# madronalabs/madronalib

Measured on AMD Instinct MI355X. Metric: voice-samples/sec (SawGen->SVF chain), higher is better.
Workload: dtype f32

## Files before the change

include/mlgpu.h:

```cpp
#ifndef MLGPU_H
#define MLGPU_H

#ifndef __HIPCC_RTC__
#include <stddef.h>
#endif
#include <stdint.h>

#ifdef __cplusplus
extern "C" {
#endif

#define MLGPU_FLOATS_PER_DSPVECTOR 64
#define MLGPU_ABI_VERSION 2


typedef enum mlgpu_status
{
  MLGPU_OK = 0,
  MLGPU_ERR_INVALID = 1,
  MLGPU_ERR_NO_DEVICE = 2,
  MLGPU_ERR_HIP = 3,
  MLGPU_ERR_OOM = 4,
  MLGPU_ERR_UNSUPPORTED = 5,
  MLGPU_ERR_RANGE = 6,
// ... 270 lines not shown
  const char* name;
  int node_type;
  int kind;
  int n_inputs;
  int n_required_inputs;
  int n_params;
  const char* output_name;
} mlgpu_registry_entry;
int mlgpu_registry_count(void);
int mlgpu_registry_get(int index, mlgpu_registry_entry* out);
int mlgpu_registry_lookup(const char* name, mlgpu_registry_entry* out);
int mlgpu_registry_input_name(const char* name, int index, char* buf, size_t buf_len);
int mlgpu_registry_param_name(const char* name, int index, char* buf, size_t buf_len);
int mlgpu_registry_param_index(const char* name, const char* param);
int mlgpu_graph_add_named(mlgpu_graph* g, const char* proc_name, const char* node_name, const char* const* input_node_names, int n_inputs);
int mlgpu_graph_set_named_coeff(mlgpu_graph* g, const char* node_name, const char* coeff_name, const float* h_per_voice, float uniform);
int mlgpu_graph_set_param_by_name(mlgpu_graph* g, const char* param_name, const float* h_per_voice, float uniform);

int mlgpu_graph_add_output(mlgpu_graph* g, int node);
int mlgpu_graph_node(mlgpu_graph* g, const char* name);
int mlgpu_graph_set_node_name(mlgpu_graph* g, int node, const char* name);
int mlgpu_graph_node_kind(mlgpu_graph* g, int node);
int mlgpu_graph_node_use_count(mlgpu_graph* g, int node);
int mlgpu_graph_num_nodes(mlgpu_graph* g);
int mlgpu_graph_set_voices_per_lane(mlgpu_graph* g, int n);
size_t mlgpu_graph_device_bytes(mlgpu_graph* g);
int mlgpu_graph_set_autotune(mlgpu_graph* g, int on);
int mlgpu_graph_tuning(mlgpu_graph* g, int* voices_per_lane, int* quads_per_trip);
int mlgpu_graph_workgroups_per_cu(mlgpu_graph* g);
int mlgpu_graph_compile(mlgpu_graph* g);
int mlgpu_graph_compile_async(mlgpu_graph* g);
int mlgpu_graph_compile_poll(mlgpu_graph* g);
const char* mlgpu_graph_source(mlgpu_graph* g);
int mlgpu_graph_emit(mlgpu_graph* g, const void** code, size_t* code_size);
const char* mlgpu_graph_last_error(mlgpu_graph* g);
int mlgpu_graph_clear(mlgpu_graph* g);
int mlgpu_graph_clear_proc(mlgpu_graph* g, int proc_node);
int mlgpu_graph_set_state_uniform(mlgpu_graph* g, int proc_node, int state_idx, uint32_t value);
int mlgpu_graph_set_param(mlgpu_graph* g, int param_node, const float* h_per_voice);
int mlgpu_graph_set_param_uniform(mlgpu_graph* g, int param_node, float value);
int mlgpu_graph_num_coeffs(mlgpu_graph* g, int proc_node);
int mlgpu_graph_num_state(mlgpu_graph* g, int proc_node);
int mlgpu_graph_set_coeff(mlgpu_graph* g, int proc_node, int coeff_idx, const float* h_per_voice);
int mlgpu_graph_set_coeff_uniform(mlgpu_graph* g, int proc_node, int coeff_idx, float value);
int mlgpu_graph_get_state(mlgpu_graph* g, int proc_node, int state_idx, uint32_t* h_per_voice);
int mlgpu_graph_set_state(mlgpu_graph* g, int proc_node, int state_idx, const uint32_t* h_per_voice);
int mlgpu_graph_process(mlgpu_graph* g, size_t n_vectors, const float* const* d_inputs, int in_layout,
                        float* const* d_outputs, int out_layout);
int mlgpu_graph_set_input_layout(mlgpu_graph* g, int input_index, int layout);
int mlgpu_graph_process_ctl(mlgpu_graph* g, size_t n_vectors, const float* const* d_inputs, int in_layout,
                            const float* const* d_controls, float* const* d_outputs, int out_layout);

int mlgpu_engine_set_jit(mlgpu_engine* e, int enabled);
int mlgpu_jit_selftest(char* log, size_t log_len);
int mlgpu_jit_stats(uint64_t* compiles, uint64_t* disk_hits, uint64_t* memory_hits, double* compile_seconds, double* disk_load_seconds);
int mlgpu_jit_cache_export(void* buffer, size_t capacity, size_t* needed);
int mlgpu_jit_cache_import(const void* buffer, size_t size, size_t* kernels);
int mlgpu_jit_cache_clear_memory(void);
int mlgpu_jit_compiler_available(void);

typedef enum mlgpu_event_type
{
  MLGPU_EVENT_NULL = 0,
  MLGPU_EVENT_NOTE_ON = 1,
  MLGPU_EVENT_NOTE_RETRIG = 2,
  MLGPU_EVENT_NOTE_SUSTAIN = 3,
// ... 157 lines not shown
```

madronalib_amd/__init__.py:

```python
import ctypes
import weakref

import numpy as np

from . import _lib
from .constants import FLOATS_PER_DSPVECTOR, Layout, Op, Proc, Region, Route, RowOp, RowsRule, Status, Vop

__all__ = ["Engine", "Bank", "Graph", "DSPBuffer", "ProcessBuffer", "Resampler", "Events", "Event", "EventType", "jit_selftest", "DeviceBuffer", "MlgpuError", "Layout", "Op", "Proc", "RowOp", "Status", "Vop", "Route", "RowsRule", "Allpass1", "FractionalDelay", "LinearGlide", "SampleAccurateLinearGlide",
           "Lopass", "Hipass", "Bandpass", "LoShelf", "HiShelf", "Bell", "OnePole", "DCBlocker", "ADSR",
           "dBToGain", "device_count", "FLOATS_PER_DSPVECTOR"]


BUSY = 7


def behaviour_revision():
    return _lib.load().mlgpu_behaviour_revision()


class MlgpuError(RuntimeError):
    def __init__(self, status, detail=""):
        L = _lib.load()
        self.status = status
        super().__init__(f"mlgpu status {status} ({L.mlgpu_status_string(status).decode()}) {detail}")
# ... 1022 lines not shown
    def add_output(self, node):
        self.outputs.append(node)
        self.engine._check(self.L.mlgpu_graph_add_output(self.h, self._id(node)))

    def set_output_group_sum(self, output_index, group):
        self._check(self.L.mlgpu_graph_set_output_group_sum(self.h, int(output_index), int(group)))

    def set_output_mixdown(self, output_index, on=True):
        self._check(self.L.mlgpu_graph_set_output_mixdown(self.h, int(output_index), 2 if on == "shard" else (1 if on else 0)))

    def reserve_mixdown(self, max_vectors):
        self._check(self.L.mlgpu_graph_reserve_mixdown(self.h, int(max_vectors)))

    def set_input_group(self, input_index, group):
        self._check(self.L.mlgpu_graph_set_input_group(self.h, int(input_index), int(group)))

    def compile(self):
        self.engine._check(self.L.mlgpu_graph_compile(self.h))

    def compile_async(self):
        self.engine._check(self.L.mlgpu_graph_compile_async(self.h))

    def compile_poll(self):
        st = self.L.mlgpu_graph_compile_poll(self.h)
        if st == BUSY:
            return False
        self.engine._check(st)
        return True

    @property
    def source(self):
        return self.L.mlgpu_graph_source(self.h).decode()

    def clear(self):
        self.engine._check(self.L.mlgpu_graph_clear(self.h))

    def set_param(self, node, value):
        if np.isscalar(value):
            self.engine._check(self.L.mlgpu_graph_set_param_uniform(self.h, self._id(node), float(value)))
        else:
            v = np.ascontiguousarray(value, np.float32)
            assert v.shape == (self.V,)
            self.engine._check(self.L.mlgpu_graph_set_param(self.h, self._id(node), _np_ptr(v)))

    def set_coeff(self, node, idx, value):
        if np.isscalar(value):
            self.engine._check(self.L.mlgpu_graph_set_coeff_uniform(self.h, self._id(node), idx, float(value)))
        else:
            v = np.ascontiguousarray(value, np.float32)
            assert v.shape == (self.V,)
            self.engine._check(self.L.mlgpu_graph_set_coeff(self.h, self._id(node), idx, _np_ptr(v)))

    def set_coeffs(self, node, coeffs):
        for i, c in enumerate(coeffs):
            self.set_coeff(node, i, c if np.ndim(c) else float(c))

    def num_state(self, node):
        return self.L.mlgpu_graph_num_state(self.h, self._id(node))

    def get_state(self, node, idx):
        out = np.empty(self.V, np.uint32)
        self.engine._check(self.L.mlgpu_graph_get_state(self.h, self._id(node), idx, _np_ptr(out)))
        return out

    def set_state(self, node, idx, value):
        v = np.ascontiguousarray(np.broadcast_to(np.asarray(value, np.uint32), (self.V,)))
# ... 145 lines not shown
```

madronalib_amd/_lib.py:

```python
import ctypes
import os
import subprocess
import threading

HERE = os.path.dirname(os.path.abspath(__file__))
CSRC = os.path.join(HERE, "csrc")
LIB_PATH = os.path.join(CSRC, "libmlgpu.so")
HEADER = os.path.join(os.path.dirname(HERE), "include", "mlgpu.h")

def _sources():
    names = {"Makefile", "embed.py"}
    try:
        text = open(os.path.join(CSRC, "Makefile")).read().replace("\\\n", " ")
        vars_ = {}
        for line in text.splitlines():
            if "=" in line and not line.startswith("\t") and not line.lstrip().startswith("#"):
                k, _, v = line.partition("=")
                vars_[k.strip().rstrip("?:+").strip()] = v.strip()
        for key in ("SRCS", "DEVHDRS", "HDRS"):
            for tok in vars_.get(key, "").split():
                if tok.startswith("$("):
                    continue
                names.add(tok)
    except OSError:
# ... 146 lines not shown
    sig("mlgpu_graph_add_const", i, [vp, f])
    sig("mlgpu_graph_set_live_constants", i, [vp, i])
    sig("mlgpu_graph_set_const", i, [vp, i, f])
    sig("mlgpu_graph_update_constants_from", i, [vp, vp])
    sig("mlgpu_graph_add_const_vector", i, [vp, ctypes.POINTER(ctypes.c_float), ctypes.c_char_p])
    sig("mlgpu_graph_add_control", i, [vp, c.c_char_p])
    sig("mlgpu_graph_add_feedback", i, [vp, c.c_char_p])
    sig("mlgpu_graph_set_feedback", i, [vp, i, i])
    sig("mlgpu_graph_set_max_delay", i, [vp, i, f])
    sig("mlgpu_allpass1_make_coeffs", f, [f])
    sig("mlgpu_fractional_delay_make_state", None, [f, fp])
    sig("mlgpu_graph_add_vop", i, [vp, i, ip, i, c.c_char_p])
    sig("mlgpu_graph_process_ctl", i, [vp, sz, pp, i, pp, pp, i])
    sig("mlgpu_graph_last_error", c.c_char_p, [vp])
    sig("mlgpu_graph_set_output_group_sum", i, [vp, i, i])
    sig("mlgpu_graph_set_output_mixdown", i, [vp, i, i])
    sig("mlgpu_graph_reserve_mixdown", i, [vp, sz])
    sig("mlgpu_graph_set_input_group", i, [vp, i, i])
    sig("mlgpu_graph_add_event_row", i, [vp, i, c.c_char_p])
    sig("mlgpu_graph_bind_events", i, [vp, vp])
    sig("mlgpu_graph_process_events", i, [vp, sz, i, pp, i, pp, pp, i])
    sig("mlgpu_linear_glide_make_coeffs", None, [f, fp])
    sig("mlgpu_sample_accurate_linear_glide_make_coeffs", None, [f, fp])
    sig("mlgpu_graph_add_proc", i, [vp, i, ip, i, c.c_char_p])
    sig("mlgpu_graph_add_op", i, [vp, i, ip, i, c.c_char_p])
    sig("mlgpu_graph_add_output", i, [vp, i])
    sig("mlgpu_graph_node", i, [vp, c.c_char_p])
    sig("mlgpu_graph_num_nodes", i, [vp])
    sig("mlgpu_graph_compile", i, [vp])
    sig("mlgpu_graph_compile_async", i, [vp])
    sig("mlgpu_graph_compile_poll", i, [vp])
    sig("mlgpu_behaviour_revision", i, [])
    sig("mlgpu_graph_source", c.c_char_p, [vp])
    sig("mlgpu_graph_node_use_count", i, [vp, i])
    sig("mlgpu_graph_emit", i, [vp, c.POINTER(vp), c.POINTER(c.c_size_t)])
    sig("mlgpu_graph_begin_region", i, [vp, i, c.POINTER(i), i, c.POINTER(i)])
    sig("mlgpu_graph_end_region", i, [vp, i, c.c_char_p])
    sig("mlgpu_graph_clear", i, [vp])
    sig("mlgpu_graph_clear_proc", i, [vp, i])
    sig("mlgpu_graph_set_input_layout", i, [vp, i, i])
    sig("mlgpu_graph_set_voices_per_lane", i, [vp, i])
    sig("mlgpu_graph_set_delay_layout", i, [vp, i])
    sig("mlgpu_graph_delay_layout", i, [vp])
    sig("mlgpu_graph_device_bytes", sz, [vp])
    sig("mlgpu_graph_set_autotune", i, [vp, i])
    sig("mlgpu_graph_tuning", i, [vp, c.POINTER(i), c.POINTER(i)])
    sig("mlgpu_graph_workgroups_per_cu", i, [vp])
    sig("mlgpu_mixdown_reserve", i, [vp, sz, sz])
    sig("mlgpu_mixdown_shard_level", i, [sz])
    sig("mlgpu_mixdown_shard_rows", sz, [sz])
    sig("mlgpu_mixdown_shard", i, [vp, vp, i, sz, sz, vp, vp])
    sig("mlgpu_bank_process_mixdown_shard", i, [vp, sz, vp, i, vp, vp])
    sig("mlgpu_mixdown_finish", i, [fp, sz, sz, i, fp, fp])
    sig("mlgpu_mixdown", i, [vp, vp, i, sz, sz, vp, vp])
    sig("mlgpu_mixdown_groups", i, [vp, vp, i, sz, sz, sz, vp, i])
    sig("mlgpu_events_create", i, [vp, sz, i, pp])
    sig("mlgpu_events_destroy", i, [vp])
    sig("mlgpu_events_clear", i, [vp])
    sig("mlgpu_events_set_sample_rate", i, [vp, c.c_double])
    sig("mlgpu_events_set_protocol", i, [vp, i])
    sig("mlgpu_events_set_unison", i, [vp, i])
    sig("mlgpu_events_set_mod_cc", i, [vp, i])
    sig("mlgpu_events_set_pitch_bend_semitones", i, [vp, f])
    sig("mlgpu_events_set_mpe_pitch_bend_semitones", i, [vp, f])
    sig("mlgpu_events_set_pitch_glide_seconds", i, [vp, f])
    sig("mlgpu_events_set_drift_amount", i, [vp, f])
# ... 80 lines not shown
```

madronalib_amd/csrc/graph.hip:

```cpp
#include <math.h>
#include <stdio.h>
#include <stdlib.h>
#include <string.h>

#include <algorithm>
#include <atomic>
#include <thread>
#include <mutex>
#include <new>
#include <set>

#include "graph_codegen.hpp"
#include "mlgpu_internal.hpp"

using namespace mlgraph;

struct mlgpu_graph;
static std::mutex g_boundMutex;
static std::set<mlgpu_graph*> g_boundGraphs;

namespace
{
int opArity(int op) { return op >= 64 ? 3 : (op >= 32 ? 2 : 1); }
bool opKnown(int op)
// ... 771 lines not shown
    {
      err = allocate(g->d_consts, (size_t)(g->desc.nConsts + 1));
      for (const Node& n : g->desc.nodes)
        if (n.type == NODE_CONST && err == hipSuccess)
        {
          uint32_t u;
          memcpy(&u, &n.value, 4);
          err = mlgpu_launch_fill32((uint32_t*)g->d_consts.get() + n.slot, u, 1, e->stream);
        }
    }
    for (const Node& n : g->desc.nodes)
    {
      if (n.type != NODE_PROC) continue;
      float dc[MLGPU_MAX_PROC_COEFFS];
      mlgpu_proc_default_coeffs(n.kind, dc);
      for (int i = 0; i < n.nc && err == hipSuccess; ++i)
      {
        uint32_t u;
        memcpy(&u, &dc[i], 4);
        if (u) err = mlgpu_launch_fill32((uint32_t*)g->d_coeffs.get() + (size_t)(n.cOff + i) * V, u, V, e->stream);
      }
      uint32_t words[MLGPU_MAX_PROC_STATE];
      mlgpu_proc_clear_state(n.kind, words, false);
      for (int i = 0; i < n.ns && err == hipSuccess; ++i)
        err = mlgpu_launch_fill32(g->d_state.get() + (size_t)(n.sOff + i) * V, words[i], V, e->stream);
    }
    if (err != hipSuccess) return gfail(g, err == hipErrorOutOfMemory ? MLGPU_ERR_OOM : MLGPU_ERR_HIP, std::string("graph_compile: ") + hipGetErrorString(err));
    g->compiled = true;
    return MLGPU_OK;
  }

  const char* mlgpu_graph_source(mlgpu_graph* g) { return (g && !g->job && g->build) ? g->build->source.c_str() : ""; }

  static int clearNode(mlgpu_graph* g, size_t node)
  {
    const Node& n = g->desc.nodes[node];
    hipError_t err = hipSetDevice(g->e->device);
    if (n.type == NODE_FEEDBACK)
    {
      for (int i = 0; i < n.ns && err == hipSuccess; ++i) err = mlgpu_launch_fill32(g->d_state.get() + (size_t)(n.sOff + i) * g->desc.V, 0u, g->desc.V, g->e->stream);
    }
    else if (n.type == NODE_PROC)
    {
      uint32_t words[MLGPU_MAX_PROC_STATE];
      mlgpu_proc_clear_state(n.kind, words, true);
      const uint64_t mask = mlgpu_proc_clear_mask(n.kind);
      for (int i = 0; i < n.ns && err == hipSuccess; ++i)
        if ((mask >> (i < 64 ? i : 63)) & 1) err = mlgpu_launch_fill32(g->d_state.get() + (size_t)(n.sOff + i) * g->desc.V, words[i], g->desc.V, g->e->stream);
      if (err == hipSuccess && n.ringLen)
        err = mlgpu_launch_fill32((uint32_t*)g->d_mem.get() + g->build->plan.nodes[node].memOff * g->build->plan.memVoices, 0u, n.ringLen * (size_t)mlgpu_proc_rings(n.kind) * g->build->plan.memVoices, g->e->stream);
    }
    if (err != hipSuccess) return gfail(g, MLGPU_ERR_HIP, hipGetErrorString(err));
    return MLGPU_OK;
  }

  int mlgpu_graph_clear(mlgpu_graph* g)
  {
    if (!g) return MLGPU_ERR_INVALID;
    if (g->job) return MLGPU_ERR_BUSY;
    if (!g->compiled) return MLGPU_ERR_INVALID;
    for (size_t node = 0; node < g->desc.nodes.size(); ++node)
    {
      const int st = clearNode(g, node);
      if (st) return st;
    }
    g->vectorCount = 0;
// ... 376 lines not shown
```

madronalib_amd/csrc/graph_codegen.cpp:

```cpp
#include "graph_codegen.hpp"

#include <stdio.h>
#include <string.h>

#include <algorithm>
#include <sstream>

using namespace mlgraph;

namespace
{
std::string floatLiteral(float f)
{
  uint32_t u;
  memcpy(&u, &f, 4);
  char buf[48];
  snprintf(buf, sizeof(buf), "u2f(0x%08xu)", u);
  return buf;
}

int upDepth(const GraphDesc& g, int r)
{
  int d = 0;
  for (; r >= 0; r = g.regions[(size_t)r].parent) d += (g.regions[(size_t)r].kind == MLGPU_REGION_UPSAMPLE_2X);
// ... 41 lines not shown
      if (streamedOsc(m, MLGPU_PROC_PULSE_GEN) && m.in[0] == n.in[0] && (m.in.size() == 1 || g.nodes[m.in[1]].rate == RATE_VOICE))
      {
        p.nodes[i].streamLockPulse = (int)j;
        p.nodes[i].streamLockSaw = p.nodes[j].streamLockSaw = (int)i;
        break;
      }
    }
  }
}

void planOscTrips(const GraphDesc& g, GraphPlan& p)
{
  for (size_t i = 0; i < g.nodes.size(); ++i)
  {
    const Node& n = g.nodes[i];
    if (p.oscTripQ <= 0 || n.type != NODE_PROC || n.region >= 0 || n.rate != RATE_AUDIO) continue;
    if (n.kind != MLGPU_PROC_SAW_GEN && n.kind != MLGPU_PROC_PULSE_GEN) continue;
    if (n.in.empty() || g.nodes[n.in[0]].rate != RATE_VOICE) continue;
    p.nodes[i].oscTrip = n.kind == MLGPU_PROC_SAW_GEN || n.in.size() == 1 || g.nodes[n.in[1]].rate == RATE_VOICE;
    p.oscTrips = p.oscTrips || p.nodes[i].oscTrip;
  }
  auto trip = [&](size_t j, int kind) { return p.nodes[j].oscTrip && g.nodes[j].kind == kind; };
  for (size_t i = 0; i < g.nodes.size(); ++i)
  {
    if (!trip(i, MLGPU_PROC_SAW_GEN)) continue;
    bool first = true;
    for (size_t k = 0; k < i; ++k) first = first && !(trip(k, MLGPU_PROC_SAW_GEN) && g.nodes[k].in[0] == g.nodes[i].in[0]);
    for (size_t j = 0; first && j < g.nodes.size(); ++j)
      if (trip(j, MLGPU_PROC_PULSE_GEN) && g.nodes[j].in[0] == g.nodes[i].in[0])
      {
        p.nodes[i].lockedPartner = (int)j;
        break;
      }
  }
}

void planEarlyReads(const GraphDesc& g, GraphPlan& p)
{
  std::vector<char> movable(g.nodes.size(), 0), wanted(g.nodes.size(), 0);
  if (!p.earlyRows) return;
  for (size_t j = 0; j < g.nodes.size(); ++j)
  {
    const Node& m = g.nodes[j];
    if (m.rate != RATE_AUDIO)
    {
      movable[j] = 1;
      continue;
    }
    bool ok = m.region < 0 && m.role == ROLE_NONE && (m.type == NODE_OP || m.type == NODE_INPUT || m.type == NODE_FEEDBACK || m.type == NODE_VOP || (m.type == NODE_PROC && !mlgpu_proc_rings(m.kind) && p.nodes[j].streamLockSaw < 0));
    if (m.type != NODE_FEEDBACK)
      for (int in : m.in) ok = ok && movable[(size_t)in];
    movable[j] = ok;
  }
  for (size_t j = 0; j < g.nodes.size(); ++j)
  {
    const Node& m = g.nodes[j];
    if (p.nodes[j].earlySlot < 0) continue;
    bool all = true;
    for (size_t a = 1; a < m.in.size(); ++a) all = all && movable[(size_t)m.in[a]];
    if (!all) continue;
    for (size_t a = 1; a < m.in.size(); ++a) wanted[(size_t)m.in[a]] = 1;
    p.nodes[j].earlyTop = true;
  }
  for (size_t j = g.nodes.size(); j-- > 0;)
  {
    const Node& m = g.nodes[j];
// ... 4 lines not shown
  }
  int after = 0;
  for (size_t b = g.nodes.size(); b-- > 0;)
    if (p.nodes[b].earlyTop)
    {
      p.nodes[b].earlyPending = after;
      after += g.nodes[b].kind == MLGPU_PROC_PITCHBENDABLE_DELAY ? 2 : 1;
    }
}

std::string nodeExpr(const GraphDesc& g, const GraphPlan& p, size_t i, int l, const std::string& ph = "", const std::string& idx = "q * 4 + k")
{
  const Node& n = g.nodes[i];
  std::ostringstream s;
  const std::string L = "_" + std::to_string(l);
  auto arg = [&](size_t j) { return "n" + std::to_string(n.in[j]) + ph.substr(0, (size_t)upDepth(g, g.nodes[n.in[j]].region)) + L; };
  auto argsFrom = [&](size_t j0) {
    std::string t;
    for (size_t j = j0; j < n.in.size(); ++j) t += ", " + arg(j);
    return t;
  };
  switch (n.type)
  {
    case NODE_INPUT: s << "xin" << n.slot << L << "[k]"; break;
    case NODE_CONTROL: s << "ctl" << n.slot << L << "[t * a.V]"; break;
    case NODE_EVENT_ROW: s << (n.slot == 0 ? "evP" : "evG") << L << "[k]"; break;
    case NODE_PARAM: s << "a.params[(size_t)" << n.slot << " * a.V + v" << L << "]"; break;
    case NODE_CONST:
      if (g.liveConsts) s << "a.consts[" << n.slot << "]";
      else s << floatLiteral(n.value);
      break;
    case NODE_PROC:
      if (ph.empty() && p.nodes[i].streamLockSaw >= 0)
        s << "sl" << p.nodes[i].streamLockSaw << (n.kind == MLGPU_PROC_SAW_GEN ? "s" : "p") << L;
      else if (n.kind == MLGPU_PROC_TEMPO_LOCK && g.nodes[n.in[0]].type != NODE_INPUT)
        s << "p" << i << L << ".next_x(" << idx << ", " << arg(0) << ", " << arg(1) << ", " << arg(2) << ")";
      else if (mlgpu_proc_is_vector_rate(n.kind))
        s << "p" << i << L << ".next_n(" << idx << ")";
      else if (p.nodes[i].earlySlot >= 0)
        s << "p" << i << L << (n.kind == MLGPU_PROC_PITCHBENDABLE_DELAY ? ".post_i<" : ".post<") << p.nodes[i].earlyPending << ">("
          << (n.kind == MLGPU_PROC_PITCHBENDABLE_DELAY ? idx + ", " : std::string()) << arg(0) << ")";
      else if (n.kind == MLGPU_PROC_PITCHBENDABLE_DELAY)
        s << "p" << i << L << ".next_i(" << idx << ", " << arg(0) << ", " << arg(1) << ((p.rings == RingLayout::SECTORS && n.region < 0) ? ", qq * 4 + k" : "") << ")";
      else if (p.rings == RingLayout::SECTORS && n.region < 0 && mlgpu_proc_rings(n.kind))
        s << "p" << i << L << ".next_k(qq * 4 + k, " << arg(0) << argsFrom(1) << ")";
      else if (p.nodes[i].oscTrip)
        s << "osc" << i << L << "[qq * 4 + k]";
      else if ((n.kind == MLGPU_PROC_SAW_GEN || n.kind == MLGPU_PROC_PULSE_GEN) && g.nodes[n.in[0]].rate == RATE_VOICE)
      {
        const bool widthSignal = n.in.size() == 2 && g.nodes[n.in[1]].rate != RATE_VOICE;
        s << "p" << i << L << (widthSignal ? ".next_uw(" : ".next_u(") << arg(0);
        if (n.in.size() == 2) s << ", " << arg(1);
        s << ", odd" << i << ")";
      }
      else if (n.kind == MLGPU_PROC_PULSE_GEN && (n.in.size() == 1 || g.nodes[n.in[1]].rate == RATE_VOICE))
      {
        s << "p" << i << L << ".next_sw(" << arg(0);
        if (n.in.size() == 2) s << ", " << arg(1);
        s << ", oddw" << i << ")";
      }
      else if (n.kind == MLGPU_PROC_PULSE_GEN && n.in.size() == 2)
        s << "p" << i << L << ".next2(" << arg(0) << ", " << arg(1) << ")";
      else
        s << "p" << i << L << ".next(" << (n.in.empty() ? std::string("0.f") : arg(0)) << argsFrom(1) << ")";
      break;
    case NODE_OP:
      if (n.kind == MLGPU_OP_CLAMP && clampHasConstBounds(g, n))
// ... 301 lines not shown
      s << "    }\n";
    }
    if (ringTrips)
      for (size_t i = 0; i < g.nodes.size(); ++i)
        if (g.nodes[i].type == NODE_PROC && g.nodes[i].region < 0 && mlgpu_proc_rings(g.nodes[i].kind))
          for (int l = 0; l < VL; ++l) s << "    p" << i << sfx(l) << ".trip_begin();\n";
    s << "#pragma unroll\n    for (int qq = 0; qq < " << tq << "; ++qq)\n    {\n      const int q = q2 + qq;\n";
  }
  void quadHead()
  {
    if (PF) s << "      const bool lastQ = (q == 15), lastT = (t + 1 == a.T);\n";
    for (int i = 0; i < g.nInputs; ++i)
      for (int l = 0; l < VL; ++l)
      {
        s << "      const f32x4 xin" << i << sfx(l) << " = nx" << i << sfx(l) << ";\n      pf" << i << sfx(l) << " += lastQ ? (lastT ? (size_t)0 : a.in[" << i
          << "].strideT - 15 * a.in[" << i << "].strideQ) : a.in[" << i << "].strideQ;\n      nx" << i << sfx(l) << " = __builtin_nontemporal_load(pf" << i << sfx(l) << ");\n";
      }
    for (size_t o = 0; o < g.outputs.size(); ++o)
      for (int l = 0; l < VL; ++l) s << "      f32x4 y" << o << sfx(l) << ";\n";
    if (g.hasEventRows)
      for (int l = 0; l < VL; ++l)
        s << "      mlev::CtlVoice::f32x4e evP" << sfx(l) << ", evG" << sfx(l) << ";\n      ev" << sfx(l) << ".quad(t, q, evP" << sfx(l) << ", evG" << sfx(l) << ");\n";
    for (size_t i = 0; i < g.nodes.size(); ++i)
      if (g.nodes[i].type == NODE_FEEDBACK && g.nodes[i].region < 0)
        for (int l = 0; l < VL; ++l)
        {
          const std::string nm = std::to_string(i) + sfx(l);
          s << "      float fbv" << nm << "[4];\n#pragma unroll\n      for (int kk = 0; kk < 4; ++kk)\n      {\n        fbv" << nm << "[kk] = fbn" << nm << "[kk];\n        fbn" << nm
            << "[kk] = fbm" << nm << "[kk];\n        fbm" << nm << "[kk] = u2f(" << stateRef(std::to_string(g.nodes[i].sOff) + " + ((q + 2) & 15) * 4 + kk", l) << ");\n      }\n";
        }
    for (size_t i = 0; i < g.nodes.size(); ++i)
      if (g.nodes[i].type == NODE_PROC && (g.nodes[i].kind == MLGPU_PROC_LINEAR_GLIDE || g.nodes[i].kind == MLGPU_PROC_HALF_BAND_BUFFERED))
        for (int l = 0; l < VL; ++l) s << "      p" << i << sfx(l) << ".begin_quad(q);\n";
    s << "#pragma unroll\n      for (int k = 0; k < 4; ++k)\n      {\n";
  }
  struct Ctx { std::string sfx, idx, vec, indent; };
  bool isInside(int r, int ancestor) const
  {
    for (; r >= 0; r = g.regions[(size_t)r].parent)
      if (r == ancestor) return true;
    return false;
  }
  int childUnder(int r, int ancestor) const
  {
    while (g.regions[(size_t)r].parent != ancestor) r = g.regions[(size_t)r].parent;
    return r;
  }
  std::string regionSource(int in, const Ctx& c, int l) const
  {
    const int src = g.nodes[(size_t)in].in[0];
    return name(src, c.sfx.substr(0, (size_t)upDepth(g, g.nodes[(size_t)src].region)), l);
  }
  void emitPre(size_t dn, const Ctx& c)
  {
    const Node& m = g.nodes[dn];
    for (int l = 0; l < VL; ++l)
    {
      s << c.indent << "p" << dn << sfx(l) << (m.kind == MLGPU_PROC_PITCHBENDABLE_DELAY ? ".pre_i(" + c.idx : ".pre(");
      for (size_t a = 1; a < m.in.size(); ++a) s << ((a > 1 || m.kind == MLGPU_PROC_PITCHBENDABLE_DELAY) ? ", " : "") << name(m.in[a], "", l);
      s << ");\n";
    }
  }
  void streamLockPair(int si, const Ctx& c)
  {
    const int pj = p.nodes[(size_t)si].streamLockPulse;
    const Node &sn = g.nodes[(size_t)si], &pn = g.nodes[(size_t)pj];
    for (int l = 0; l < VL; ++l)
// ... 18 lines not shown
      for (size_t j = 0; j < g.nodes.size(); ++j)
        if (p.nodes[j].earlyHoisted) value(j, c.indent, c.sfx, c.idx);
      for (size_t dn = 0; dn < g.nodes.size(); ++dn)
        if (p.nodes[dn].earlyTop) emitPre(dn, c);
    }
    for (size_t j = 0; j < g.nodes.size(); ++j)
    {
      const Node& m = g.nodes[j];
      if (m.rate != RATE_AUDIO) continue;
      if (r < 0 && p.earlyRows && p.nodes[j].earlyHoisted) continue;
      if (m.region != r)
      {
        if (m.region >= 0 && (r < 0 || isInside(m.region, r)))
        {
          const int child = childUnder(m.region, r);
          if (!entered[(size_t)child])
          {
            entered[(size_t)child] = 1;
            emitRegion(child, c);
          }
        }
        continue;
      }
      if (m.role == ROLE_REGION_IN) continue;
      if (m.role == ROLE_REGION_OUT)
      {
        const Region& R = g.regions[(size_t)m.slot];
        if (R.kind == MLGPU_REGION_DOWNSAMPLE_2X) continue;
        for (int l = 0; l < VL; ++l)
          s << c.indent << "const float " << name((int)j, c.sfx, l) << " = p" << j << sfx(l) << ".down(" << name(m.in[0], c.sfx + "a", l) << ", "
            << name(m.in[0], c.sfx + "b", l) << ");" << (l == 0 && !m.name.empty() ? "  // " + m.name : std::string()) << "\n";
        continue;
      }
      if (r < 0 && p.nodes[j].streamLockSaw >= 0)
      {
        const int si = p.nodes[j].streamLockSaw;
        if ((int)j == std::min(si, p.nodes[(size_t)si].streamLockPulse)) streamLockPair(si, c);
      }
      if (r < 0 && p.nodes[j].earlySlot >= 0 && !p.nodes[j].earlyTop) emitPre(j, c);
      value(j, c.indent, c.sfx, c.idx);
    }
    if (r < 0) return;
    for (size_t j = 0; j < g.nodes.size(); ++j)
      if (g.nodes[j].region == r && g.nodes[j].type == NODE_FEEDBACK && g.nodes[j].fbSource >= 0)
        for (int l = 0; l < VL; ++l)
          s << c.indent << stateRef(std::to_string(g.nodes[j].sOff) + " + " + c.idx, l) << " = f2u(" << name(g.nodes[j].fbSource, c.sfx, l) << ");\n";
    bool any = false;
    for (size_t j = 0; j < g.nodes.size(); ++j)
    {
      const Node& m = g.nodes[j];
      if (m.type != NODE_PROC || m.region != r || m.role != ROLE_NONE) continue;
      if (!any) s << c.indent << "if (" << c.idx << " == 63)\n" << c.indent << "{\n";
      any = true;
      for (int l = 0; l < VL; ++l) s << c.indent << "  p" << j << sfx(l) << ".end_vector();\n";
    }
    if (any) s << c.indent << "}\n";
  }
  void emitRegion(int r, const Ctx& c)
  {
    const Region& R = g.regions[(size_t)r];
    if (R.kind == MLGPU_REGION_UPSAMPLE_2X)
    {
      for (int phase = 0; phase < 2; ++phase)
      {
        const std::string ph = phase ? "b" : "a";
        const Ctx cc{c.sfx + ph, "((2 * (" + c.idx + ") + " + std::to_string(phase) + ") & 63)",
                     "(2 * (" + c.vec + ") + ((2 * (" + c.idx + ") + " + std::to_string(phase) + ") >> 6))", c.indent};
// ... 148 lines not shown
  if (p.rings == RingLayout::WINDOWS && ldsLayout1 + ldsOther > kLdsBytes)
    return fail(MLGPU_ERR_UNSUPPORTED, "graph_compile: delay layouts 1 and 4 need 8 KiB of LDS per ring (" + kib(ldsLayout1) + " for " + std::to_string(p.totalRings) +
                                           " rings) next to " + kib(ldsOther) + " of output strips and tables; a workgroup has 160 KiB");
  if (ldsOther > kLdsBytes)
    return fail(MLGPU_ERR_UNSUPPORTED, "graph_compile: " + kib(ldsOther) + " of LDS for the outputs summed inside the kernel (21 KiB per mixed-down output, 20.3 KiB per 16-voice group sum); a workgroup has 160 KiB");
  p.memVoices = p.rings != RingLayout::ROWS ? ((g.V + 255) & ~(size_t)255) : g.V;
  p.minWavesHook = hooks.minWaves;
  p.rowAddr64 = hooks.rowAddr64;
  p.rowAddr32 = p.rings == RingLayout::ROWS && p.totalRings && g.V < ((size_t)1 << 22) && !p.rowAddr64;
  if (p.rings == RingLayout::ROWS && p.totalRings && hooks.earlyReads)
  {
    int slots = 0;
    for (const Node& n : g.nodes)
      if (n.type == NODE_PROC && n.region < 0 && n.role == ROLE_NONE && mlgpu_proc_rings(n.kind)) slots += n.kind == MLGPU_PROC_PITCHBENDABLE_DELAY ? 2 : 1;
    if (slots >= 3 && (size_t)slots * 4 * 64 * sizeof(float) + ldsOther <= kLdsBytes)
    {
      p.earlyRows = true;
      p.earlySlots = slots;
      slots = 0;
      for (size_t i = 0; i < g.nodes.size(); ++i)
      {
        const Node& n = g.nodes[i];
        if (n.type != NODE_PROC || n.region >= 0 || n.role != ROLE_NONE || !mlgpu_proc_rings(n.kind)) continue;
        p.nodes[i].earlySlot = slots;
        slots += n.kind == MLGPU_PROC_PITCHBENDABLE_DELAY ? 2 : 1;
      }
    }
  }
  planStreamLocks(g, p);
  planEarlyReads(g, p);
  p.oscTripQ = hooks.oscTripQ;
  if (p.rings == RingLayout::SECTORS && p.totalRings && p.oscTripQ > 0) p.oscTripQ = 2;
  planOscTrips(g, p);
  p.form = KernelForm{graphVoicesPerLane(g), (p.totalRings && p.rings == RingLayout::ROWS) ? 2 : 1, 0};
  return MLGPU_OK;
}

std::string mlgraph::generateGraphSource(const GraphDesc& d, const GraphPlan& plan, const KernelForm& form)
{
  GraphEmitter e(d, plan, form);
  e.header();
  e.sharedMemory();
  e.voiceSetup();
  e.oscillatorTests();
  e.outputsAndPrefetch();
  e.vectorHead();
  e.sampleBody();
  e.outputStores();
  e.epilogue();
  return e.s.str();
}
```

madronalib_amd/csrc/graph_codegen.hpp:

```cpp
#pragma once
#include <stddef.h>
#include <stdint.h>

#include <string>
#include <vector>

#include "../../include/mlgpu.h"

int mlgpu_proc_rings(int kind);
bool mlgpu_proc_is_vector_rate(int kind);

constexpr int kHostMixStripFloats = 64 * 20 + 3 * 16 + 16;
constexpr int kHostGroup16StripFloats = 4 * (4 * 80 + 4);
constexpr int kHostTurnClockShift = 13;
constexpr int kHostGraphMaxInputs = 32, kHostGraphMaxOutputs = 8;

namespace mlgraph
{
enum NodeType
{
  NODE_INPUT = 0,
  NODE_PARAM = 1,
  NODE_CONST = 2,
  NODE_PROC = 3,
// ... 56 lines not shown
  int nInputs{0}, nParams{0}, nControls{0}, nConsts{0}, NC{0}, NS{0};
  bool hasImpulse{false};
  bool hasEventRows{false};
  bool strictSvf{false};
  bool liveConsts{false};
  int delayLayout{0};
  int voicesPerLane{0};
  bool autotune{false};
};

enum class RingLayout
{
  ROWS = 0,
  WINDOWS,
  TRANSPOSED,
  SECTORS
};
inline int apiLayout(RingLayout r) { return r == RingLayout::SECTORS ? 4 : (int)r; }
inline RingLayout ringLayoutOfApi(int layout) { return layout == 4 ? RingLayout::SECTORS : layout == 3 ? RingLayout::WINDOWS : (RingLayout)layout; }

struct KernelForm
{
  int voicesPerLane{1}, quadsPerTrip{1}, minWaves{0};
};

struct TestHooks
{
  int minWaves{-1};
  bool rowAddr64{false};
  bool earlyReads{true};
  int oscTripQ{2};
};

struct NodePlan
{
  size_t memOff{0};
  int ringSlot{0};
  int earlySlot{-1};
  bool earlyTop{false};
  int earlyPending{0};
  bool earlyHoisted{false};
  bool oscTrip{false};
  int lockedPartner{-1};
  int streamLockPulse{-1};
  int streamLockSaw{-1};
};

struct GraphPlan
{
  RingLayout rings{RingLayout::ROWS};
  int totalRings{0};
  size_t memFloatsPerVoice{0};
  size_t memVoices{0};
  bool rowAddr32{false};
  bool rowAddr64{false};
  bool earlyRows{false};
  int earlySlots{0};
  int oscTripQ{2};
  bool oscTrips{false};
  int minWavesHook{-1};
  KernelForm form;
  std::vector<NodePlan> nodes;
};

int planGraph(const GraphDesc& d, const TestHooks& hooks, GraphPlan& plan, std::string& error);

std::string generateGraphSource(const GraphDesc& d, const GraphPlan& plan, const KernelForm& form);
}
```

madronalib_amd/csrc/mldsp_procs.hpp:

```cpp
#pragma once
#include "mldsp_math.hpp"
#ifdef __HIPCC_RTC__
#include "mlgpu.h"
#else
#include "../../include/mlgpu.h"
#endif

namespace mldev
{
struct VoiceMem
{
  const float* coeffs;
  uint32_t* state;
  size_t V;
  float* mem{nullptr};
  uint32_t memMask{0};
  MLD float* ringPtr(int ringIdx, uint32_t i) const
  {
    if (addr32) return (float*)((char*)(mem + (size_t)((uint32_t)ringIdx * (memMask + 1)) * V) + (__umul24(i, V4) + lane4));
    return mem + (size_t)((uint32_t)ringIdx * (memMask + 1) + i) * V;
  }
  MLD float ring(int ringIdx, uint32_t i) const { return *ringPtr(ringIdx, i); }
  MLD void ringSet(int ringIdx, uint32_t i, float x) const { *ringPtr(ringIdx, i) = x; }
  float* lds{nullptr};
// ... 2163 lines not shown
  }
  return false;
}

template <bool REGULAR_W>
MLD void step_locked_stream(Proc<MLGPU_PROC_SAW_GEN>& saw, Proc<MLGPU_PROC_PULSE_GEN>& pulse, float cps, float w, float& outSaw, float& outPulse)
{
  const float p = phasor_next(saw.omega32, cps);
  pulse.omega32 = saw.omega32;
  const float sawv = __builtin_fmaf(p, 2.f, -1.f);
  const float pulsev = (p >= w) ? -1.f : 1.f;
  const float d = p - w + 1.0f;
  const float down = REGULAR_W ? __builtin_amdgcn_fractf(d) : d - (float)sse_cvtt(d);
  const bool downOdd = !REGULAR_W && !(abs_ps(down) <= 2.0f);
  const BlepFreq<false> f = BlepFreq<false>::make(cps, downOdd);
  const bool loUp = f.lo(p), nearUp = loUp || f.hi(p);
  const bool loDown = f.lo(down), nearDown = loDown || f.hi(down);
  outSaw = sawv;
  outPulse = pulsev;
  if (__builtin_amdgcn_ballot_w64(nearUp || nearDown) == 0) return;
  const bool full = f.anyLaneOdd();
  if (__builtin_amdgcn_ballot_w64(nearUp && nearDown) == 0)
  {
    const float c = f.correction(nearDown ? down : p, nearDown ? loDown : loUp, full);
    outPulse = nearDown ? (pulsev - c) : (nearUp ? (pulsev + c) : pulsev);
    outSaw = nearUp ? (sawv - c) : sawv;
    return;
  }
  const float cUp = f.correction(p, loUp, full), cDown = f.correction(down, loDown, full);
  outPulse = (pulsev + (nearUp ? cUp : 0.f)) - (nearDown ? cDown : 0.f);
  outSaw = sawv - (nearUp ? cUp : 0.f);
}

template <class P, class = void>
struct HasFastPath
{
  static constexpr bool value = false;
};
template <class P>
struct HasFastPath<P, decltype((void)&P::input_is_odd)>
{
  static constexpr bool value = true;
};

template <int... KINDS>
struct Chain;

template <>
struct Chain<>
{
  static constexpr int NC = 0, NS = 0;
  static constexpr bool kHasImpulse = false;
  MLD void load(VoiceMem, const KernelTables&) {}
  MLD void store(VoiceMem) const {}
  MLD float next(float x) { return x; }
  MLD void end_vector() {}
  static constexpr bool kHeadHasFastPath = false;
  static MLD bool head_input_is_odd(float) { return false; }
  template <bool FAST>
  MLD float next_head(float x)
  {
    return x;
  }
};

template <int K0, int... KS>
// ... 47 lines not shown
```

Measured before the change: 1321 billion.

## Generate saw and pulse oscillators four samples at a time with wave-uniform fast path

Adds a planning pass that marks saw and pulse generators whose frequency inputs can be computed ahead, then emits code that evaluates those inputs for a quad of samples and runs the oscillator over the quad. When a wave-wide ballot shows no lane is near a discontinuity, the oscillator skips the per-sample band-limiting correction and emits the naive saw or pulse directly. Otherwise it falls back to the per-sample path. This trades some extra registers for the quad arrays and an added ballot check against cheaper per-sample oscillator work. It also adds an API call that reports each oscillator's chosen form.

```diff
diff --git a/include/mlgpu.h b/include/mlgpu.h
--- a/include/mlgpu.h
+++ b/include/mlgpu.h
@@ -326,6 +326,7 @@
 int mlgpu_graph_compile_async(mlgpu_graph* g);
 int mlgpu_graph_compile_poll(mlgpu_graph* g);
 const char* mlgpu_graph_source(mlgpu_graph* g);
+int mlgpu_graph_osc_form(mlgpu_graph* g, int node);
 int mlgpu_graph_emit(mlgpu_graph* g, const void** code, size_t* code_size);
 const char* mlgpu_graph_last_error(mlgpu_graph* g);
 int mlgpu_graph_clear(mlgpu_graph* g);
diff --git a/madronalib_amd/__init__.py b/madronalib_amd/__init__.py
--- a/madronalib_amd/__init__.py
+++ b/madronalib_amd/__init__.py
@@ -1078,6 +1078,9 @@
     def source(self):
         return self.L.mlgpu_graph_source(self.h).decode()
 
+    def osc_form(self, node):
+        return (None, "per sample", "quad", "trip")[self._ret(self.L.mlgpu_graph_osc_form(self.h, self._id(node)), None)]
+
     def clear(self):
         self.engine._check(self.L.mlgpu_graph_clear(self.h))
 
diff --git a/madronalib_amd/_lib.py b/madronalib_amd/_lib.py
--- a/madronalib_amd/_lib.py
+++ b/madronalib_amd/_lib.py
@@ -202,6 +202,7 @@
     sig("mlgpu_graph_compile_poll", i, [vp])
     sig("mlgpu_behaviour_revision", i, [])
     sig("mlgpu_graph_source", c.c_char_p, [vp])
+    sig("mlgpu_graph_osc_form", i, [vp, i])
     sig("mlgpu_graph_node_use_count", i, [vp, i])
     sig("mlgpu_graph_emit", i, [vp, c.POINTER(vp), c.POINTER(c.c_size_t)])
     sig("mlgpu_graph_begin_region", i, [vp, i, c.POINTER(i), i, c.POINTER(i)])
diff --git a/madronalib_amd/csrc/graph.hip b/madronalib_amd/csrc/graph.hip
--- a/madronalib_amd/csrc/graph.hip
+++ b/madronalib_amd/csrc/graph.hip
@@ -827,6 +827,19 @@
 
   const char* mlgpu_graph_source(mlgpu_graph* g) { return (g && !g->job && g->build) ? g->build->source.c_str() : ""; }
 
+  int mlgpu_graph_osc_form(mlgpu_graph* g, int node)
+  {
+    if (!g) return -MLGPU_ERR_INVALID;
+    if (g->job) return -MLGPU_ERR_BUSY;
+    if (node < 0 || node >= (int)g->desc.nodes.size()) return -MLGPU_ERR_RANGE;
+    if (g->build) return g->build->plan.nodes[(size_t)node].oscForm;
+    GraphPlan plan;
+    std::string error;
+    const int st = planGraph(g->desc, readTestHooks(), plan, error);
+    if (st != MLGPU_OK) return -gfail(g, st, error);
+    return plan.nodes[(size_t)node].oscForm;
+  }
+
   static int clearNode(mlgpu_graph* g, size_t node)
   {
     const Node& n = g->desc.nodes[node];
diff --git a/madronalib_amd/csrc/graph_codegen.cpp b/madronalib_amd/csrc/graph_codegen.cpp
--- a/madronalib_amd/csrc/graph_codegen.cpp
+++ b/madronalib_amd/csrc/graph_codegen.cpp
@@ -97,6 +97,43 @@
         p.nodes[i].lockedPartner = (int)j;
         break;
       }
+  }
+}
+
+void planOscForms(const GraphDesc& g, GraphPlan& p)
+{
+  std::vector<char> ahead(g.nodes.size(), 0);
+  for (size_t j = 0; j < g.nodes.size(); ++j)
+  {
+    const Node& m = g.nodes[j];
+    if (m.rate != RATE_AUDIO)
+      ahead[j] = m.type != NODE_PROC;
+    else if (m.region < 0 && m.role == ROLE_NONE && (m.type == NODE_INPUT || m.type == NODE_EVENT_ROW))
+      ahead[j] = 1;
+    else if (m.region < 0 && m.role == ROLE_NONE && m.type == NODE_OP)
+    {
+      ahead[j] = 1;
+      for (int in : m.in) ahead[j] = ahead[j] && ahead[(size_t)in];
+    }
+  }
+  std::vector<char> wanted(g.nodes.size(), 0);
+  for (size_t i = 0; i < g.nodes.size(); ++i)
+  {
+    const Node& n = g.nodes[i];
+    if (n.type != NODE_PROC || (n.kind != MLGPU_PROC_SAW_GEN && n.kind != MLGPU_PROC_PULSE_GEN)) continue;
+    p.nodes[i].oscForm = p.nodes[i].oscTrip ? OSC_TRIP : OSC_PER_SAMPLE;
+    if (p.nodes[i].oscTrip || p.earlyRows || n.region >= 0 || n.rate != RATE_AUDIO || n.in.empty()) continue;
+    const Node& f = g.nodes[(size_t)n.in[0]];
+    if (f.rate == RATE_VOICE || !ahead[(size_t)n.in[0]]) continue;
+    if (n.kind == MLGPU_PROC_PULSE_GEN && n.in.size() == 2 && g.nodes[(size_t)n.in[1]].rate != RATE_VOICE) continue;
+    p.nodes[i].oscForm = OSC_QUAD;
+    wanted[(size_t)n.in[0]] = 1;
+  }
+  for (size_t j = g.nodes.size(); j-- > 0;)
+  {
+    if (!wanted[j] || g.nodes[j].rate != RATE_AUDIO) continue;
+    p.nodes[j].quadAhead = true;
+    for (int in : g.nodes[j].in) wanted[(size_t)in] = 1;
   }
 }
 
@@ -167,7 +204,9 @@
       break;
     case NODE_PROC:
       if (ph.empty() && p.nodes[i].streamLockSaw >= 0)
-        s << "sl" << p.nodes[i].streamLockSaw << (n.kind == MLGPU_PROC_SAW_GEN ? "s" : "p") << L;
+        s << "sl" << p.nodes[i].streamLockSaw << (n.kind == MLGPU_PROC_SAW_GEN ? "s" : "p") << L << (p.nodes[i].oscForm == OSC_QUAD ? "[k]" : "");
+      else if (ph.empty() && p.nodes[i].oscForm == OSC_QUAD)
+        s << "oq" << i << L << "[k]";
       else if (n.kind == MLGPU_PROC_TEMPO_LOCK && g.nodes[n.in[0]].type != NODE_INPUT)
         s << "p" << i << L << ".next_x(" << idx << ", " << arg(0) << ", " << arg(1) << ", " << arg(2) << ")";
       else if (mlgpu_proc_is_vector_rate(n.kind))
@@ -535,7 +574,57 @@
     for (size_t i = 0; i < g.nodes.size(); ++i)
       if (g.nodes[i].type == NODE_PROC && (g.nodes[i].kind == MLGPU_PROC_LINEAR_GLIDE || g.nodes[i].kind == MLGPU_PROC_HALF_BAND_BUFFERED))
         for (int l = 0; l < VL; ++l) s << "      p" << i << sfx(l) << ".begin_quad(q);\n";
+    quadOscillators();
     s << "#pragma unroll\n      for (int k = 0; k < 4; ++k)\n      {\n";
+  }
+  void quadOscillators()
+  {
+    bool any = false;
+    for (size_t j = 0; j < g.nodes.size(); ++j) any = any || p.nodes[j].quadAhead;
+    for (size_t j = 0; j < g.nodes.size(); ++j)
+      if (p.nodes[j].quadAhead)
+        for (int l = 0; l < VL; ++l) s << "      float qa" << j << sfx(l) << "[4];\n";
+    if (any) s << "#pragma unroll\n      for (int k = 0; k < 4; ++k)\n      {\n";
+    for (size_t j = 0; j < g.nodes.size(); ++j)
+      if (p.nodes[j].quadAhead)
+      {
+        value(j, "        ");
+        for (int l = 0; l < VL; ++l) s << "        qa" << j << sfx(l) << "[k] = " << name((int)j, "", l) << ";\n";
+      }
+    if (any) s << "      }\n";
+    for (size_t i = 0; i < g.nodes.size(); ++i)
+    {
+      const Node& n = g.nodes[i];
+      if (p.nodes[i].oscForm != OSC_QUAD) continue;
+      const int si = p.nodes[i].streamLockSaw, pj = si >= 0 ? p.nodes[(size_t)si].streamLockPulse : -1;
+      if (si >= 0 && (int)i != std::min(si, pj)) continue;
+      for (int l = 0; l < VL; ++l)
+      {
+        std::string freq = "qa" + std::to_string(n.in[0]) + sfx(l);
+        if (g.nodes[(size_t)n.in[0]].rate != RATE_AUDIO)
+        {
+          freq = "qf" + std::to_string(i) + sfx(l);
+          s << "      const float " << freq << "[4] = {" << name(n.in[0], "", l) << ", " << name(n.in[0], "", l) << ", " << name(n.in[0], "", l) << ", " << name(n.in[0], "", l) << "};\n";
+        }
+        if (si >= 0)
+        {
+          const std::string S = "sl" + std::to_string(si) + "s" + sfx(l), P = "sl" + std::to_string(si) + "p" + sfx(l), w = width((size_t)pj, l);
+          const std::string ps = "p" + std::to_string(si) + sfx(l), pp = "p" + std::to_string(pj) + sfx(l);
+          s << "      float " << S << "[4], " << P << "[4];\n";
+          s << "      if (slocked" << si << " && !oddw" << pj << ") quad_locked_stream(" << ps << ", " << pp << ", " << freq << ", " << w << ", " << S << ", " << P << ");\n";
+          s << "      else\n      {\n#pragma unroll\n        for (int k = 0; k < 4; ++k)\n        {\n";
+          s << "          if (slocked" << si << ") step_locked_stream<false>(" << ps << ", " << pp << ", " << freq << "[k], " << w << ", " << S << "[k], " << P << "[k]);\n";
+          s << "          else\n          {\n            " << S << "[k] = " << ps << ".next(" << freq << "[k]);\n            " << P << "[k] = " << pp << ".next_sw(" << freq << "[k], " << w << ", oddw" << pj << ");\n          }\n";
+          s << "        }\n      }\n";
+        }
+        else
+        {
+          s << "      float oq" << i << sfx(l) << "[4];\n      quad_stream(p" << i << sfx(l) << ", " << freq;
+          if (n.kind == MLGPU_PROC_PULSE_GEN) s << ", " << width(i, l) << ", oddw" << i;
+          s << ", oq" << i << sfx(l) << ");\n";
+        }
+      }
+    }
   }
   struct Ctx { std::string sfx, idx, vec, indent; };
   bool isInside(int r, int ancestor) const
@@ -620,7 +709,12 @@
             << name(m.in[0], c.sfx + "b", l) << ");" << (l == 0 && !m.name.empty() ? "  // " + m.name : std::string()) << "\n";
         continue;
       }
-      if (r < 0 && p.nodes[j].streamLockSaw >= 0)
+      if (r < 0 && p.nodes[j].quadAhead)
+      {
+        for (int l = 0; l < VL; ++l) s << c.indent << "const float " << name((int)j, "", l) << " = qa" << j << sfx(l) << "[k];\n";
+        continue;
+      }
+      if (r < 0 && p.nodes[j].streamLockSaw >= 0 && p.nodes[j].oscForm != OSC_QUAD)
       {
         const int si = p.nodes[j].streamLockSaw;
         if ((int)j == std::min(si, p.nodes[(size_t)si].streamLockPulse)) streamLockPair(si, c);
@@ -835,6 +929,7 @@
   p.oscTripQ = hooks.oscTripQ;
   if (p.rings == RingLayout::SECTORS && p.totalRings && p.oscTripQ > 0) p.oscTripQ = 2;
   planOscTrips(g, p);
+  planOscForms(g, p);
   p.form = KernelForm{graphVoicesPerLane(g), (p.totalRings && p.rings == RingLayout::ROWS) ? 2 : 1, 0};
   return MLGPU_OK;
 }
diff --git a/madronalib_amd/csrc/graph_codegen.hpp b/madronalib_amd/csrc/graph_codegen.hpp
--- a/madronalib_amd/csrc/graph_codegen.hpp
+++ b/madronalib_amd/csrc/graph_codegen.hpp
@@ -112,6 +112,14 @@
   int oscTripQ{2};
 };
 
+enum OscForm
+{
+  OSC_NONE = 0,
+  OSC_PER_SAMPLE = 1,
+  OSC_QUAD = 2,
+  OSC_TRIP = 3
+};
+
 struct NodePlan
 {
   size_t memOff{0};
@@ -124,6 +132,8 @@
   int lockedPartner{-1};
   int streamLockPulse{-1};
   int streamLockSaw{-1};
+  int oscForm{OSC_NONE};
+  bool quadAhead{false};
 };
 
 struct GraphPlan
diff --git a/madronalib_amd/csrc/mldsp_procs.hpp b/madronalib_amd/csrc/mldsp_procs.hpp
--- a/madronalib_amd/csrc/mldsp_procs.hpp
+++ b/madronalib_amd/csrc/mldsp_procs.hpp
@@ -2219,6 +2219,69 @@
   outSaw = sawv - (nearUp ? cUp : 0.f);
 }
 
+constexpr uint32_t kQuadMaxStep = 1u << 28;
+constexpr uint32_t kQuadSlack = 1024u;
+MLD uint32_t quad_step_bound(const float (&cps)[4])
+{
+  uint32_t S = 0u;
+#pragma unroll
+  for (int k = 0; k < 4; ++k) S = trip_umax(S, (uint32_t)sse_cvt(cps[k] * kStepsPerCycle));
+  return S;
+}
+MLD bool quad_step_is_dense(uint32_t S) { return S > kQuadMaxStep; }
+MLD bool quad_near_step(uint32_t c0, uint32_t S) { return (c0 + 5u * S + kQuadSlack) < (6u * S + 2u * kQuadSlack); }
+MLD uint32_t pulse_width_steps(float w) { return (w < 1.0f) ? (uint32_t)(w * kStepsPerCycle) : 0u; }
+
+MLD void quad_stream(Proc<MLGPU_PROC_SAW_GEN>& saw, const float (&cps)[4], float (&out)[4])
+{
+  const uint32_t S = quad_step_bound(cps);
+  if (__builtin_amdgcn_ballot_w64(quad_step_is_dense(S) || quad_near_step(saw.omega32, S)) == 0)
+  {
+#pragma unroll
+    for (int k = 0; k < 4; ++k) out[k] = __builtin_fmaf(phasor_next_hi(saw.omega32, cps[k]), 2.f * kPhaseUnit, -1.f);
+    return;
+  }
+#pragma unroll
+  for (int k = 0; k < 4; ++k) out[k] = saw.next(cps[k]);
+}
+
+MLD void quad_stream(Proc<MLGPU_PROC_PULSE_GEN>& pulse, const float (&cps)[4], float w, bool oddW, float (&out)[4])
+{
+  if (!oddW)
+  {
+    const uint32_t S = quad_step_bound(cps), c0 = pulse.omega32;
+    if (__builtin_amdgcn_ballot_w64(quad_step_is_dense(S) || quad_near_step(c0, S) || quad_near_step(c0 - pulse_width_steps(w), S)) == 0)
+    {
+      const float wS = w * kPhaseScale;
+#pragma unroll
+      for (int k = 0; k < 4; ++k) out[k] = (phasor_next_hi(pulse.omega32, cps[k]) >= wS) ? -1.f : 1.f;
+      return;
+    }
+  }
+#pragma unroll
+  for (int k = 0; k < 4; ++k) out[k] = pulse.next_sw(cps[k], w, oddW);
+}
+
+MLD void quad_locked_stream(Proc<MLGPU_PROC_SAW_GEN>& saw, Proc<MLGPU_PROC_PULSE_GEN>& pulse, const float (&cps)[4], float w, float (&outSaw)[4], float (&outPulse)[4])
+{
+  const uint32_t S = quad_step_bound(cps), c0 = saw.omega32;
+  if (__builtin_amdgcn_ballot_w64(quad_step_is_dense(S) || quad_near_step(c0, S) || quad_near_step(c0 - pulse_width_steps(w), S)) == 0)
+  {
+    const float wS = w * kPhaseScale;
+#pragma unroll
+    for (int k = 0; k < 4; ++k)
+    {
+      const float h = phasor_next_hi(saw.omega32, cps[k]);
+      outSaw[k] = __builtin_fmaf(h, 2.f * kPhaseUnit, -1.f);
+      outPulse[k] = (h >= wS) ? -1.f : 1.f;
+    }
+    pulse.omega32 = saw.omega32;
+    return;
+  }
+#pragma unroll
+  for (int k = 0; k < 4; ++k) step_locked_stream<true>(saw, pulse, cps[k], w, outSaw[k], outPulse[k]);
+}
+
 template <class P, class = void>
 struct HasFastPath
 {
```

Result: no change. 1322 billion, median of 2 (+0.1%).
